# thawro/pytorch-human-pose

Measured on AMD Instinct MI355X. Metric: images/sec (fwd+decode) HigherHRNet-W32 512px, higher is better.
Workload: dtype bf16; 1 GPU; HigherHRNet-W32 inference bf16, batch 32 @ 512x512 per GPU (conv fwd on N(0,1) images + AE decode on constructed maps, 10 people/image, det_thr 0.05, tag_thr 0.5, adjust+refine); global_batch=32, parallelism=image-sharded replicas x1, no data-path collective

## Files before the change

include/hhrnet.h:

```cpp
#ifndef HHRNET_H
#define HHRNET_H
#include <stdint.h>

#ifdef __cplusplus
extern "C" {
#endif

#define HH_ABI_VERSION 3
#define HH_DTYPE_BF16 1
#define HH_DTYPE_FP8 2
#define HH_DTYPE_F16 3

typedef struct hh_net hh_net;
typedef struct hh_decoder hh_decoder;

int hh_abi_version(void);
const char *hh_last_error(void);

hh_net *hh_create(int num_kpts, int C, int dtype);
void hh_destroy(hh_net *net);

hh_net *hh_create_classifier(int C, int num_classes, int dtype);
int hh_forward_classifier(hh_net *net, const float *images, int B, int H, int W, float *logits, void *stream);

int hh_num_params(const hh_net *net);
const char *hh_param_name(const hh_net *net, int index);
int hh_param_shape(const hh_net *net, int index, int64_t shape[4]);

int hh_load_weights(hh_net *net, const char *name, const float *host, const int64_t *shape, int ndim);
int hh_finalize(hh_net *net);

int hh_calibrate(hh_net *net, const float *images, int B, int H, int W, int rounds, void *stream);

int hh_e4m3_encode(const float *x, int64_t n, unsigned char *out);
int hh_e4m3_decode(const unsigned char *x, int64_t n, float *out);

int hh_reserve(hh_net *net, int B, int H, int W);
int64_t hh_workspace_bytes(const hh_net *net);

int hh_forward(hh_net *net, const float *images, int B, int H, int W, float *init_heatmaps, float *deconv_heatmaps,
               int use_graph, void *stream);

int hh_set_multi_lane(hh_net *net, int enable);

int hh_debug_check_plan(const hh_net *net);

double hh_forward_flops(const hh_net *net, int B, int H, int W);

int hh_profile_enable(hh_net *net, int enable);
int hh_profile_count(const hh_net *net);
int hh_profile_get(hh_net *net, int index, int *cfg, double *flops, double *bytes, float *ms, float *kernel_ms, const char **layer);
int hh_profile_clock(hh_net *net, int index, double *ghz);
int hh_conv_config(int cfg, int out[7]);
int hh_conv_config_double_buffered(int cfg);

int hh_debug_conv_bench(int cfg, int B, int Hin, int Win, int cin, int cout, int with_res, int relu, int iters,
                        float *ms_per_launch, unsigned long long *stamps16, int ref_cfg, float *max_diff);

int hh_debug_bb_bench(int B, int H, int W, int iters, float *ms_per_launch, unsigned long long *stamps64);
int hh_debug_bb_compare(int B, int H, int W, int iters, float *max_diff, float *ms_classic, float *ms_pc);

int hh_debug_bb_cover(int B, int H, int W, int tall, int num_cus, int64_t counts[4]);

int hh_set_taps(hh_net *net, int enable);
int hh_num_taps(const hh_net *net);
const char *hh_tap_name(const hh_net *net, int index);
int hh_tap_shape(const hh_net *net, int index, int64_t shape[4]);
int hh_tap_read(hh_net *net, int index, float *host_nchw);

int hh_preprocess_u8(const unsigned char *image_hwc, int h, int w, const double dst_to_src[6], float *out_nchw, int H, int W,
                     const float mean[3], const float stdv[3], void *stream);

typedef struct hh_image_desc {
    long long offset;
    int h, w;
    double dst_to_src[6];
} hh_image_desc;
int hh_preprocess_u8_batch(const unsigned char *images_base, const hh_image_desc *descs_dev, int n, float *out_nchw, int H, int W,
                           const float mean[3], const float stdv[3], void *stream);

int hh_flip_images(const float *images, float *out, int B, int C, int H, int W, void *stream);
int hh_flip_merge(float *hm, int64_t hm_bstride, const float *hm_flipped, int64_t hmf_bstride, const float *tags_flipped,
                  int64_t tf_bstride, float *tags_out, int64_t to_bstride, const int32_t *perm_host, int B, int K,
                  int h, int w, void *stream);

hh_decoder *hh_decoder_create(int num_kpts, int max_people, double det_thr, double tag_thr);
void hh_decoder_destroy(hh_decoder *dec);
int hh_decoder_reserve(hh_decoder *dec, int B, int H, int W, int E);
int hh_decoder_set_exact_topk(hh_decoder *dec, int enable);

#define HH_DECODE_FALLBACK 1
#define HH_DECODE_SOLVER_GUARD 2
int hh_decode(hh_decoder *dec, const float *hm_q, int64_t hm_q_bstride, const float *hm_h, int64_t hm_h_bstride,
              const float *const *tags_q, const int64_t *tags_bstride, int E, int B, int hq, int wq, int adjust,
              int refine, float *joints, float *scores, int32_t *num_people, int32_t *flags, void *stream);

int hh_parse(hh_decoder *dec, const float *hm_full, const float *tags_full, int E, int B, int H, int W, int adjust,
             int refine, float *joints, float *scores, int32_t *num_people, int32_t *flags, void *stream);

int hh_loss_heatmaps(const float *pred, int64_t pred_bstride, const float *target, const float *mask, int B, int K, int h, int w,
                     float *loss, float *grad, int64_t grad_bstride, double *scratch, void *stream);
int hh_loss_ae_grouping(const float *tags, int64_t tags_bstride, const int32_t *joints, const int32_t *num_people, int B, int P, int K,
                        int h, int w, float *push_pull, float *grad, int64_t grad_bstride, float push_scale, float pull_scale,
                        double *scratch, void *stream);

#define HH_TRAIN_MAX_STAGES 4
typedef struct hh_train_desc {
    long long image_offset, mask_offset;
    int h, w;
    int flip, reserved;
    double image_dst_to_src[6];
    double mask_dst_to_src[HH_TRAIN_MAX_STAGES][6];
} hh_train_desc;
int hh_train_images_u8_batch(const unsigned char *batch_base, const hh_train_desc *descs_dev, int n, float *out_nchw, int H, int W,
                             const float mean[3], const float stdv[3], void *stream);
int hh_train_masks_u8_batch(const unsigned char *batch_base, const hh_train_desc *descs_dev, int n, int nstages, const int *stage_hw,
                            float *const *out, void *stream);
#define HH_MOSAIC_MAX_S 8192
typedef struct hh_mosaic_tile {
    long long image_offset, mask_offset;
    int h, w;
} hh_mosaic_tile;
typedef struct hh_mosaic_desc {
    hh_mosaic_tile tile[4];
    long long canvas_image_offset, canvas_mask_offset;
} hh_mosaic_desc;
int hh_mosaic_u8_batch(unsigned char *batch_base, const hh_mosaic_desc *descs_dev, const hh_mosaic_desc *descs_host, int n, int S,
                       void *stream);
typedef struct hh_crowd_mask_desc {
    long long mask_offset;
    int h, w;
    int seg_first, seg_count;
} hh_crowd_mask_desc;
typedef struct hh_crowd_seg_desc {
    long long toggle_offset;
    int count;
    int col_first, col_last;
    int reserved;
} hh_crowd_seg_desc;
long long hh_crowd_polygon_capacity(const double *xy, int k, int h, int w);
long long hh_crowd_polygon_toggles(const double *xy, int k, int h, int w, unsigned int *out, long long capacity);
int hh_crowd_masks_u8_batch(unsigned char *batch_base, const hh_crowd_mask_desc *descs_dev, const hh_crowd_seg_desc *segs_dev,
                            const hh_crowd_mask_desc *descs_host, const hh_crowd_seg_desc *segs_host, const unsigned char *host_base, int n,
                            int num_segs, void *stream);
int hh_crowd_mask_config(int out[4]);
// ... 403 lines not shown
```

pytorch-human-pose_amd/csrc/capi.cpp:

```cpp
#include <algorithm>
#include <cmath>
#include <cstdint>
#include <cstring>
#include <string>
#include <vector>

#include "../../include/hhrnet.h"
#include "engine.h"
#include "optim_math.h"
#include "grad_stats_math.h"
#include "ema_math.h"
#include "render_math.h"
#include "text_math.h"
#include "seg_overlay_math.h"
#include "panel_math.h"
#include "coco_eval_math.h"
#include "pose_score_math.h"
#include "cls_score_math.h"
#include "crowd_mask_math.h"
#include "track_math.h"
#include "jpeg_math.h"
#include "jpeg_dec_math.h"

const char *hh_get_error();
// ... 65 lines not shown
}
void hh_destroy(hh_net *net) { delete net; }

int hh_num_params(const hh_net *net) { return (int)net->params.size(); }
const char *hh_param_name(const hh_net *net, int i) { return (i >= 0 && i < (int)net->params.size()) ? net->params[i].name.c_str() : nullptr; }
int hh_param_shape(const hh_net *net, int i, int64_t shape[4])
{
    if (i < 0 || i >= (int)net->params.size()) return -1;
    const auto &s = net->params[i].shape;
    for (size_t d = 0; d < s.size(); ++d) shape[d] = s[d];
    return (int)s.size();
}

int hh_load_weights(hh_net *net, const char *name, const float *host, const int64_t *shape, int ndim)
{
    auto it = net->param_index.find(name);
    if (it == net->param_index.end()) { hh_set_error(std::string("hh_load_weights: unexpected key ") + name); return 1; }
    ParamSlot &p = net->params[it->second];
    if (p.counter) { p.loaded = true; return 0; }
    if (ndim != (int)p.shape.size()) { hh_set_error(std::string("hh_load_weights: rank mismatch for ") + name); return 1; }
    size_t n = 1;
    for (int d = 0; d < ndim; ++d) {
        if (shape[d] != p.shape[d]) { hh_set_error(std::string("hh_load_weights: size mismatch for ") + name); return 1; }
        n *= (size_t)shape[d];
    }
    p.data.assign(host, host + n);
    p.loaded = true;
    net->finalized = false;
    return 0;
}
int hh_e4m3_encode(const float *x, int64_t n, unsigned char *out)
{
    for (int64_t i = 0; i < n; ++i) out[i] = hh_f32_to_e4m3(x[i]);
    return 0;
}
int hh_e4m3_decode(const unsigned char *x, int64_t n, float *out)
{
    for (int64_t i = 0; i < n; ++i) out[i] = hh_e4m3_to_f32(x[i]);
    return 0;
}
int hh_finalize(hh_net *net) { return net->finalize(); }
int hh_calibrate(hh_net *net, const float *images, int B, int H, int W, int rounds, void *stream)
{
    if (!images || B <= 0 || H <= 0 || W <= 0 || H % 32 || W % 32) { hh_set_error("hh_calibrate: need images [B,3,H,W] with H, W multiples of 32"); return 1; }
    return net->calibrate(images, B, H, W, rounds > 0 ? rounds : 2, (hipStream_t)stream);
}
int hh_reserve(hh_net *net, int B, int H, int W) { return net->reserve(B, H, W); }
int64_t hh_workspace_bytes(const hh_net *net) { return net->ws_bytes; }

int hh_forward(hh_net *net, const float *images, int B, int H, int W, float *init_heatmaps, float *deconv_heatmaps,
               int use_graph, void *stream)
{
    if (net->kind != 0) { hh_set_error("hh_forward: classifier handle, use hh_forward_classifier"); return 1; }
    if (!images || !init_heatmaps || !deconv_heatmaps) { hh_set_error("hh_forward: null buffer"); return 1; }
    if (B <= 0 || H <= 0 || W <= 0 || H % 32 || W % 32) { hh_set_error("hh_forward: H and W must be positive multiples of 32"); return 1; }
    return net->forward(images, B, H, W, init_heatmaps, deconv_heatmaps, use_graph, (hipStream_t)stream);
}
double hh_forward_flops(const hh_net *net, int B, int H, int W) { return net->flops(B, H, W); }

int hh_set_multi_lane(hh_net *net, int enable)
{
    net->multi_lane = enable != 0;
    for (auto &g : net->graphs) hipGraphExecDestroy(g.exec);
    net->graphs.clear();
    return 0;
}
int hh_set_taps(hh_net *net, int enable) { net->taps_enabled = enable != 0; return 0; }
int hh_num_taps(const hh_net *net) { return (int)net->taps.size(); }
const char *hh_tap_name(const hh_net *net, int i) { return (i >= 0 && i < (int)net->taps.size()) ? net->taps[i].name.c_str() : nullptr; }
int hh_tap_shape(const hh_net *net, int i, int64_t shape[4])
{
    if (i < 0 || i >= (int)net->taps.size()) return 1;
    const TensorDesc &d = net->tensors[net->taps[i].tensor];
    shape[0] = net->lastB; shape[1] = net->taps[i].C; shape[2] = net->lastH >> d.shift; shape[3] = net->lastW >> d.shift;
    return 0;
}
int hh_tap_read(hh_net *net, int index, float *host_nchw) { return hh_tap_read_impl(net, index, host_nchw); }

int hh_debug_check_plan(const hh_net *net)
{
    std::string why;
    if (net->check_plan(&why)) { hh_set_error("schedule hazard: " + why); return 1; }
    return 0;
}

int hh_profile_enable(hh_net *net, int enable) { net->prof_enabled = enable != 0; net->prof_clk = enable == 2; net->prof_used = 0; return 0; }
int hh_profile_count(const hh_net *net) { return (int)net->prof_used; }
int hh_profile_get(hh_net *net, int i, int *cfg, double *flops, double *bytes, float *ms, float *kernel_ms, const char **layer)
{
    if (i < 0 || i >= (int)net->prof_used) { hh_set_error("hh_profile_get: index out of range"); return 1; }
    const ProfRecord &r = net->prof[i];
    HH_CHECK_HIP(hipEventSynchronize(r.e1));
    HH_CHECK_HIP(hipEventElapsedTime(ms, r.e0, r.e1));
    *cfg = r.cfg; *flops = r.flops; *bytes = r.bytes;
    *layer = net->layers[net->ops[r.op].layer].conv.c_str();
    *kernel_ms = -1.f;
    if (r.slot >= 0 && net->prof_clk && net->d_clk && net->clk_khz > 0) {
        unsigned long long t[2];
        HH_CHECK_HIP(hipMemcpy(t, net->d_clk + 4 * r.slot, 16, hipMemcpyDeviceToHost));
        if (t[1] > t[0]) *kernel_ms = (float)((double)(t[1] - t[0]) / net->clk_khz);
    }
    return 0;
}
int hh_profile_clock(hh_net *net, int i, double *ghz)
{
    if (i < 0 || i >= (int)net->prof_used) { hh_set_error("hh_profile_clock: index out of range"); return 1; }
    const ProfRecord &r = net->prof[i];
    *ghz = 0.0;
    if (r.slot >= 0 && net->prof_clk && net->d_clk && net->clk_khz > 0) {
        unsigned long long t[2];
        HH_CHECK_HIP(hipEventSynchronize(r.e1));
        HH_CHECK_HIP(hipMemcpy(t, net->d_clk + 4 * r.slot + 2, 16, hipMemcpyDeviceToHost));
        if (t[1]) *ghz = (double)t[0] / (double)t[1] * net->clk_khz * 1e-6;
    }
    return 0;
}
int hh_conv_config(int cfg, int out[7])
{
    if (cfg >= 1000 && cfg - 1000 < conv_fp8_num_configs()) {
        const Fp8ConvConfig &c = conv_fp8_config(cfg - 1000);
        out[0] = c.KS; out[1] = c.S; out[2] = c.KC; out[3] = c.NT; out[4] = 1; out[5] = c.PT; out[6] = c.TW;
        return 0;
    }
    if (cfg < 0 || cfg >= conv_num_configs()) return 1;
    const ConvConfig &c = conv_config(cfg);
    out[0] = c.KS; out[1] = c.S; out[2] = c.KC; out[3] = c.NT; out[4] = c.WC; out[5] = c.PT; out[6] = c.TW;
    return 0;
}

int hh_conv_config_double_buffered(int cfg)
{
    if (cfg >= 1000 && cfg - 1000 < conv_fp8_num_configs()) return 0;
    if (cfg < 0 || cfg >= conv_num_configs()) return -1;
    return conv_config(cfg).DB;
}

int hh_preprocess_u8(const unsigned char *image_hwc, int h, int w, const double dst_to_src[6], float *out_nchw, int H, int W,
                     const float mean[3], const float stdv[3], void *stream)
{
    if (!image_hwc || !out_nchw || h <= 0 || w <= 0 || H <= 0 || W <= 0) { hh_set_error("hh_preprocess_u8: bad argument"); return 1; }
    HH_CHECK_HIP(launch_preprocess(image_hwc, h, w, dst_to_src, out_nchw, H, W, mean, stdv, (hipStream_t)stream));
    return 0;
}

int hh_preprocess_u8_batch(const unsigned char *images_base, const hh_image_desc *descs_dev, int n, float *out_nchw, int H, int W,
                           const float mean[3], const float stdv[3], void *stream)
{
    if (!images_base || !descs_dev || !out_nchw || n <= 0 || n > 65535 || H <= 0 || W <= 0) { hh_set_error("hh_preprocess_u8_batch: bad argument"); return 1; }
    HH_CHECK_HIP(launch_preprocess_batch(images_base, descs_dev, n, out_nchw, H, W, mean, stdv,
                                         (hipStream_t)stream));
    return 0;
}

int hh_train_images_u8_batch(const unsigned char *batch_base, const hh_train_desc *descs_dev, int n, float *out_nchw, int H, int W,
                             const float mean[3], const float stdv[3], void *stream)
{
    if (!batch_base || !descs_dev || !out_nchw || !mean || !stdv) { hh_set_error("hh_train_images_u8_batch: null pointer"); return 1; }
    if (n <= 0 || n > 65535 || H <= 0 || W <= 0 || (int64_t)H * W > (1 << 30)) { hh_set_error("hh_train_images_u8_batch: need 0 < n <= 65535 and 0 < H * W <= 2^30"); return 1; }
    HH_CHECK_HIP(launch_train_images(batch_base, descs_dev, n, out_nchw, H, W, mean, stdv, (hipStream_t)stream));
    return 0;
}

int hh_train_masks_u8_batch(const unsigned char *batch_base, const hh_train_desc *descs_dev, int n, int nstages, const int *stage_hw,
                            float *const *out, void *stream)
{
    if (!batch_base || !descs_dev || !stage_hw || !out) { hh_set_error("hh_train_masks_u8_batch: null pointer"); return 1; }
// ... 2205 lines not shown
```

pytorch-human-pose_amd/csrc/kernels.h:

```cpp
#pragma once
#include <hip/hip_runtime.h>
#include <stdint.h>

#include <hip/hip_ext.h>

#include "../../include/hhrnet.h"

typedef uint16_t bf16_raw;

struct LaunchProbe { hipEvent_t start = nullptr, stop = nullptr; };
LaunchProbe &hh_launch_probe();
#define HH_LAUNCH(kernel, grid, block, lds, stream, ...)                                                            \
    do {                                                                                                            \
        LaunchProbe &lp_ = hh_launch_probe();                                                                       \
        if (lp_.start) {                                                                                            \
            hipExtLaunchKernelGGL(kernel, grid, block, lds, stream, lp_.start, lp_.stop, 0, __VA_ARGS__);           \
            lp_ = LaunchProbe{};                                                                                    \
        } else {                                                                                                    \
            hipLaunchKernelGGL(kernel, grid, block, lds, stream, __VA_ARGS__);                                      \
        }                                                                                                           \
    } while (0)

struct ConvParams {
    const bf16_raw *in;
// ... 125 lines not shown
    float *fin_out;
    int fin_K;
    unsigned long long *stamps;
    unsigned long long *clk;
};
constexpr int BBPC_TH = 14, BBPC_TW = 32;
struct BBGeom { int b, oy0, ox0; };
__host__ __device__ inline int bbpc_band(int i, int ntiles, unsigned grid)
{
    return ((ntiles & 7) == 0 && (grid & 7) == 0) ? (i & 7) * (ntiles >> 3) + (i >> 3) : i;
}
__host__ __device__ __forceinline__ BBGeom bbpc_geom(int tb, int tiles_x, int tiles_per_img, int VH)
{
    const int u = tb / tiles_per_img, tt = tb % tiles_per_img;
    const int oy = (tt / tiles_x) * BBPC_TH, bq = oy / VH;
    return BBGeom{u + bq, oy - bq * VH, (tt % tiles_x) * BBPC_TW};
}
__host__ __device__ __forceinline__ int bbpc_rowmap(int b, int y, int B, int H, int VH)
{
    const bool wrap = y >= VH;
    const int ya = wrap ? y - VH : y, bb = wrap ? b + 1 : b;
    return (((unsigned)ya < (unsigned)H) & (bb < B)) ? bb * H + ya : -1;
}
__host__ __device__ inline bool bbpc_patch_wrap(int yy, int VH) { return yy >= VH; }
__host__ __device__ inline bool bbpc_patch_row(int yy, bool wrap, bool next, int H, int VH)
{
    return ((unsigned)(wrap ? yy - VH : yy) < (unsigned)H) & (!wrap | next);
}
bool bbpc_cover(int B, int H, int W, int tall, int num_cus, long long counts[4]);

#define HH_PROF_SLOTS 1024
#define HH_CFG_BB_FUSED 100
hipError_t bb_fused_init();
hipError_t bb_fused_launch(BBParams p, int num_cus, hipStream_t s);
hipError_t bbpc_init();
bool bbpc_supported(const BBParams &p);
bool bbpc_final_supported(const BBParams &p);
hipError_t bbpc_launch(BBParams p, int num_cus, hipStream_t s, int act_dtype = 0);
#define HH_CFG_BB64_FUSED 103
hipError_t bb64_fused_init();
hipError_t bb64_fused_launch(BBParams p, int num_cus, hipStream_t s, int act_dtype = 0);

struct JuncParams {
    const bf16_raw *t2; int t2_cs;
    const bf16_raw *res; int res_cs;
    const bf16_raw *x; int x_cs;
    const bf16_raw *t2a; int t2a_cs;
    const bf16_raw *w3a; const float *b3a;
    const bf16_raw *w3, *wd, *w1;
    const float *b3, *bd, *b1;
    bf16_raw *y; int y_cs;
    bf16_raw *t1; int t1_cs;
    int npix;
    unsigned long long *clk;
};
#define HH_CFG_JUNCTION 101
hipError_t junction_init();
hipError_t junction_launch(const JuncParams &p, int num_cus, hipStream_t s, int act_dtype = 0);

struct StemParams {
    const float *images;
    const bf16_raw *w;
    const float *bias;
    bf16_raw *out; int out_cs;
    int B, H, W;
    unsigned long long *clk;
    unsigned char *out_fp8;
    float out_inv_scale;
    unsigned *absmax;
};
#define HH_CFG_STEM 102
hipError_t stem_conv_launch(const StemParams &p, hipStream_t s);
struct StemFusedParams {
    const float *images;
    const bf16_raw *w1;
    const float *b1;
    const bf16_raw *w2;
    const float *b2;
    bf16_raw *out; int out_cs;
    int B, H, W;
    unsigned long long *clk;
};
#define HH_CFG_STEM_FUSED 106
hipError_t stem_fused_init();
bool stem_fused_supported(const StemFusedParams &p);
hipError_t stem_fused_launch(const StemFusedParams &p, int num_cus, hipStream_t s, int act_dtype = 0);


struct UpAddParams {
    const bf16_raw *base; int base_cs, base_coff;
    const bf16_raw *up[3]; int up_cs[3]; int up_shift[3]; int nup;
    bf16_raw *out; int out_cs, out_coff;
    int B, H, W, C, relu;
};
hipError_t launch_upadd(const UpAddParams &p, hipStream_t s, int act_dtype = 0);
struct FusionUpParams {
    const bf16_raw *x0; int x0_cs;
    const bf16_raw *src[3];
    int src_cs[3];
    const bf16_raw *w[3];
    const float *bias[3];
    int nsrc;
    bf16_raw *out; int out_cs;
    int B, H, W;
    int tiles_x, tiles_y;
    unsigned long long *clk;
};
#define HH_CFG_FUSION_UP 107
bool fusion_up_supported(int C, int nsrc);
hipError_t fusion_up_launch(FusionUpParams p, hipStream_t s, int act_dtype = 0);
hipError_t launch_upadd_backward(const bf16_raw *dy, const bf16_raw *out, int relu, int B, int H, int W, int C, bf16_raw *g, bf16_raw *const *dup,
                                 const int *up_shift, int nup, hipStream_t s, int act_dtype = 0);
struct UpAddFp8Params {
    const unsigned char *base; int base_cs; float base_scale;
    const unsigned char *up[3]; int up_cs[3]; int up_shift[3]; float up_scale[3]; int nup;
    const bf16_raw *base16; int base16_cs;
    const bf16_raw *up16[3]; int up16_cs[3];
    unsigned char *out; int out_cs;
    float out_inv_scale;
    bf16_raw *out16; int out16_cs;
    int B, H, W, C, relu;
    unsigned *absmax;
};
hipError_t launch_upadd_fp8(const UpAddFp8Params &p, hipStream_t s);
hipError_t launch_quant_fp8(const bf16_raw *in, int in_cs, unsigned char *out, int out_cs, size_t npix, int C, float inv_scale, unsigned *absmax,
                            hipStream_t s);

hipError_t launch_lds_poison(int num_cus, hipStream_t s);
hipError_t launch_avgpool(const bf16_raw *in, int in_cs, float *out, int B, int HW, int C, hipStream_t s, int act_dtype = 0);
hipError_t launch_linear(const float *x, const float *w, const float *bias, float *y, int B, int K, int N, hipStream_t s);
hipError_t launch_avgpool_backward(const float *g, bf16_raw *dx, int B, int HW, int C, hipStream_t s, int act_dtype = 0);
hipError_t launch_linear_backward(const float *x, const float *w, const float *dy, int B, int K, int N, float *dx, float *dw, float *db,
                                  hipStream_t s);
static_assert(sizeof(hh_xent_result) == 16, "ABI 3");
hipError_t launch_softmax_xent(const float *logits, const long long *targets, int B, int N, float *dlogits, hh_xent_result *result, hipStream_t s);

static_assert(sizeof(hh_image_desc) == 64, "ABI 3");
hipError_t launch_preprocess_batch(const unsigned char *base, const hh_image_desc *descs, int n, float *out, int H, int W,
                                   const float mean[3], const float stdv[3], hipStream_t s);
hipError_t launch_warp_affine_u8(const unsigned char *img, int h, int w, const double inv[6], unsigned char *out, int H, int W, hipStream_t s);
hipError_t launch_preprocess(const unsigned char *img, int h, int w, const double inv[6], float *out, int H, int W,
                             const float mean[3], const float stdv[3], hipStream_t s);
static_assert(sizeof(hh_train_desc) == 272, "ABI 3");
struct TrainMaskStages { float *out[HH_TRAIN_MAX_STAGES]; int h[HH_TRAIN_MAX_STAGES], w[HH_TRAIN_MAX_STAGES], n; };
hipError_t launch_train_images(const unsigned char *base, const hh_train_desc *descs, int n, float *out, int H, int W, const float mean[3],
                               const float stdv[3], hipStream_t s);
hipError_t launch_train_masks(const unsigned char *base, const hh_train_desc *descs, int n, const TrainMaskStages &st, hipStream_t s);
static_assert(sizeof(hh_crop_desc) == 56, "ABI 3");
hipError_t launch_resized_crop(const unsigned char *base, const hh_crop_desc *descs, int n, float *out, int H, int W, const float mean[3],
                               const float stdv[3], hipStream_t s);
static_assert(sizeof(hh_mosaic_tile) == 24 && sizeof(hh_mosaic_desc) == 112, "ABI 3");
hipError_t launch_mosaic(unsigned char *base, const hh_mosaic_desc *descs, int n, int S, hipStream_t s);
hipError_t launch_render_poses(unsigned char *base, const hh_render_desc *descs, const hh_render_prim *prims, int n, int max_tiles, hipStream_t s);
void render_debug_host(const unsigned char *src, unsigned char *dst, const hh_render_desc &d, const hh_render_prim *prims);
hipError_t launch_resize_u8(const unsigned char *src, int h, int w, int channels, unsigned char *dst, int H, int W, hipStream_t s);
hipError_t launch_resize_u8_scaled(const unsigned char *src, int h, int w, int channels, unsigned char *dst, int H, int W, double fx, double fy, hipStream_t s);
hipError_t launch_text_labels(unsigned char *base, const hh_text_desc *descs, const hh_text_prim *prims, const uint8_t *atlas, const void *tiles,
                              long long num_tiles, hipStream_t s);
void text_debug_host(unsigned char *frame, const hh_text_desc &d, const hh_text_prim *prims, const uint8_t *atlas, const void *tiles, long long num_tiles);
hipError_t launch_seg_overlay(unsigned char *base, const hh_seg_desc *descs, const int32_t *shapes, const unsigned int *toggles, int n, int max_tiles, hipStream_t s);
hipError_t launch_jpeg_encode(unsigned char *base, const hh_jpeg_desc *descs, int n, int max_mcus, int max_rows, unsigned char *ws, int32_t *lengths,
                              hipStream_t s);
template <class Desc>
hipError_t launch_jpeg_decode(unsigned char *base, const Desc *descs, int n, int max_seg, int max_blk, int max_h, int max_w, unsigned char *ws,
                              int32_t *status, hipStream_t s);
hipError_t launch_jpeg_index(unsigned char *base, const hh_jpeg_dec_desc *descs, int n, int mps, int subseq_bytes, int32_t *status, hipStream_t s);
// ... 96 lines not shown
```

pytorch-human-pose_amd/csrc/stem_fused.hip:

```cpp
#include "mfma_dev.h"

namespace {
constexpr int T2H = 2, T2W = 32;
constexpr int MR = 2 * T2H + 1, MC = 2 * T2W + 1;
constexpr int MPIX = MR * MC, NQ = (MPIX + 31) / 32;
constexpr int PRW = 4 * T2H + 3, PCW = 4 * T2W + 3;
constexpr int PLANE = PRW * PCW, NVAL = 3 * PLANE;
constexpr int NLD = (NVAL + 255) / 256;
constexpr int PS2 = 144, HALF = (MC + 1) / 2;
constexpr int MID_BYTES = MR * 2 * HALF * PS2;
constexpr int PATCH_BYTES = ((NVAL + 1) * 2 + 15) / 16 * 16;
constexpr int OFF_PATCH = MID_BYTES, OFF_BIAS = OFF_PATCH + PATCH_BYTES, LDS_BYTES = OFF_BIAS + 2 * 64 * 4;
constexpr int RD = 3, NFB = RD + 1;
}

template <typename E>
__global__ __launch_bounds__(256, 1) void stem_fused_kernel(const StemFusedParams p)
{
    extern __shared__ __attribute__((aligned(16))) char smem[];
    unsigned short *patch = reinterpret_cast<unsigned short *>(smem + OFF_PATCH);
    const int tid = threadIdx.x;
    if (p.clk && tid == 0) atomicMin(p.clk, wall_clock64());
    const int lds0 = (int)(size_t)(__attribute__((address_space(3))) char *)smem;
    const int wave = __builtin_amdgcn_readfirstlane(tid >> 6), lane = tid & 63, r = lane & 31, h = lane >> 5;
    const int H1 = p.H >> 1, W1 = p.W >> 1, H2 = p.H >> 2, W2 = p.W >> 2;
    const size_t img_elems = (size_t)3 * p.H * p.W, out_elems = (size_t)H2 * W2 * p.out_cs;
    constexpr unsigned OOB = 0x80000000u;

    const int row2 = wave >> 1, ct2 = wave & 1;
    u32x4 a1[2][2];
#pragma unroll
    for (int ct = 0; ct < 2; ++ct)
#pragma unroll
        for (int kk = 0; kk < 2; ++kk) a1[ct][kk] = reinterpret_cast<const u32x4 *>(p.w1)[((ct * 2 + kk) * 2 + h) * 32 + r];
    u32x4 w2r[36];
    {
        const auto rs_w = __builtin_amdgcn_make_buffer_rsrc(const_cast<bf16_raw *>(p.w2), 0, 9 * 8 * 64 * 16, 0x00020000);
        static_for<36>([&](auto fc) {
            constexpr int f = decltype(fc)::value, tap = f >> 2, kk = f & 3;
            w2r[f] = __builtin_bit_cast(u32x4, __builtin_amdgcn_raw_buffer_load_b128(rs_w, (((tap * 8 + kk * 2 + h) * 64) + ct2 * 32 + r) * 16, 0, 0));
        });
    }
    if (tid < 64) {
        reinterpret_cast<float *>(smem + OFF_BIAS)[tid] = p.b1[tid];
        reinterpret_cast<float *>(smem + OFF_BIAS)[64 + tid] = p.b2[tid];
    }
    if (tid == 0) patch[NVAL] = 0;
    auto bias_acc = [&](int off) {
        f32x16 b0;
#pragma unroll
        for (int q = 0; q < 4; ++q) {
            const float4 bv = *reinterpret_cast<const float4 *>(smem + OFF_BIAS + (off + 8 * q + 4 * h) * 4);
            b0[4 * q + 0] = bv.x; b0[4 * q + 1] = bv.y; b0[4 * q + 2] = bv.z; b0[4 * q + 3] = bv.w;
        }
        return b0;
    };

    const int tiles_x = (W2 + T2W - 1) / T2W, tiles_y = (H2 + T2H - 1) / T2H, ntiles = p.B * tiles_x * tiles_y;
    struct Geom { int b, oy0, ox0; };
    auto geom = [&](int t) {
        const int tx = t % tiles_x, ty = (t / tiles_x) % tiles_y;
        return Geom{t / (tiles_x * tiles_y), ty * T2H, tx * T2W};
    };
    float pv[NLD];
    auto patch_load = [&](int t) {
        const bool on = t < ntiles;
        const Geom g = geom(on ? t : 0);
        const auto rs_img = __builtin_amdgcn_make_buffer_rsrc(const_cast<float *>(p.images + (size_t)g.b * img_elems), 0, (int)(img_elems * 4), 0x00020000);
        const int iy0 = 4 * g.oy0 - 3, ix0 = 4 * g.ox0 - 3;
#pragma unroll
        for (int it = 0; it < NLD; ++it) {
            const int i = tid + 256 * it;
            const int c = i / PLANE, rem = i - c * PLANE, py = rem / PCW, px = rem - py * PCW;
            const int iy = iy0 + py, ix = ix0 + px;
            const bool ok = on & (i < NVAL) & ((unsigned)iy < (unsigned)p.H) & ((unsigned)ix < (unsigned)p.W);
            const unsigned voff = ok ? (unsigned)(((c * p.H + iy) * p.W + ix) * 4) : OOB;
            pv[it] = __builtin_bit_cast(float, __builtin_amdgcn_raw_buffer_load_b32(rs_img, (int)voff, 0, 0));
        }
    };
    auto patch_write = [&]() {
#pragma unroll
        for (int it = 0; it < NLD; ++it) {
            const int i = tid + 256 * it;
            if (it + 1 < NLD || i < NVAL) patch[i] = E::cvt(pv[it]);
        }
    };
    int off[2][8];
#pragma unroll
    for (int kk = 0; kk < 2; ++kk)
#pragma unroll
        for (int j = 0; j < 8; ++j) {
            const int t = kk * 16 + 8 * h + j;
            off[kk][j] = t < 27 ? (t / 9) * PLANE + ((t % 9) / 3) * PCW + (t % 3) : -1;
        }

    int t = blockIdx.x;
    patch_load(t);
    patch_write();
    __syncthreads();

    for (; t < ntiles; t += gridDim.x) {
        const Geom g = geom(t);
        patch_load(t + (int)gridDim.x);

        constexpr int NQW = (NQ + 3) / 4;
        u32x4 bf[NQW][2];
#pragma unroll
        for (int qi = 0; qi < NQW; ++qi) {
            const int q = wave + 4 * qi;
            const int m = q * 32 + r, mc = m < MPIX ? m : MPIX - 1;
            const int my = mc / MC, mx = mc - my * MC;
            const int base = (2 * my) * PCW + 2 * mx;
#pragma unroll
            for (int kk = 0; kk < 2; ++kk) {
                unsigned short v[8];
#pragma unroll
                for (int j = 0; j < 8; ++j) v[j] = patch[off[kk][j] >= 0 ? base + off[kk][j] : NVAL];
                bf[qi][kk] = u32x4{(unsigned)v[0] | ((unsigned)v[1] << 16), (unsigned)v[2] | ((unsigned)v[3] << 16),
                                   (unsigned)v[4] | ((unsigned)v[5] << 16), (unsigned)v[6] | ((unsigned)v[7] << 16)};
            }
        }
        const f32x16 bias1[2] = {bias_acc(0), bias_acc(32)};
#pragma unroll
        for (int qi = 0; qi < NQW; ++qi) {
            const int q = wave + 4 * qi;
            if (q >= NQ) break;
            const int m = q * 32 + r, mc = m < MPIX ? m : MPIX - 1;
            const int my = mc / MC, mx = mc - my * MC;
            const int gy = 2 * g.oy0 - 1 + my, gx = 2 * g.ox0 - 1 + mx;
            const bool inside = ((unsigned)gy < (unsigned)H1) & ((unsigned)gx < (unsigned)W1);
            char *dst = smem + ((my * 2 + (mx & 1)) * HALF + (mx >> 1)) * PS2 + h * 16;
#pragma unroll
            for (int ct = 0; ct < 2; ++ct) {
                f32x16 acc = bias1[ct];
#pragma unroll
                for (int kk = 0; kk < 2; ++kk)
                    acc = E::mfma(a1[ct][kk], bf[qi][kk], acc);
                u32x4 o[2];
                pack_rows16<E>(acc, o);
                if (m < MPIX) {
                    *reinterpret_cast<u32x4 *>(dst + ct * 64) = inside ? o[0] : u32x4{0u, 0u, 0u, 0u};
                    *reinterpret_cast<u32x4 *>(dst + ct * 64 + 32) = inside ? o[1] : u32x4{0u, 0u, 0u, 0u};
                }
            }
        }
        __syncthreads();

        patch_write();

        {
            f32x16 acc = bias_acc(64 + ct2 * 32);
            const int ma = lds0 + (row2 * 4 * HALF + r) * PS2 + h * 16;
            u32x4 fb[NFB];
            auto ldb = [&](auto sc, int buf) {
                constexpr int s = decltype(sc)::value, tap = s >> 2, kk = s & 3, ky = tap / 3, kx = tap % 3;
                fb[buf] = lds_read_async<((ky * 2 + (kx & 1)) * HALF + (kx >> 1)) * PS2 + kk * 32>(ma);
            };
            static_for<RD>([&](auto sc) { ldb(sc, decltype(sc)::value); });
            static_for<36>([&](auto sc) {
                constexpr int s = decltype(sc)::value;
                if constexpr (s + RD < 36) ldb(std::integral_constant<int, s + RD>{}, (s + RD) % NFB);
                lds_wait<(35 - s < RD ? 35 - s : RD)>(fb[s % NFB]);
                acc = E::mfma(w2r[s], fb[s % NFB], acc);
            });
            u32x4 o[2];
            pack_rows16<E>(acc, o);
            const int oy = g.oy0 + row2, ox = g.ox0 + r;
            const bool ok = (oy < H2) & (ox < W2);
            const auto rs_out = __builtin_amdgcn_make_buffer_rsrc(p.out + (size_t)g.b * out_elems, 0, (int)(out_elems * 2), 0x00020000);
            const unsigned voff = ok ? (unsigned)(((oy * W2 + ox) * p.out_cs + ct2 * 32 + 8 * h) * 2) : OOB;
            __builtin_amdgcn_raw_buffer_store_b128(o[0], rs_out, (int)voff, 0, 0);
            __builtin_amdgcn_raw_buffer_store_b128(o[1], rs_out, (int)voff, 32, 0);
        }
        __syncthreads();
    }
    if (p.clk && tid == 0) atomicMax(p.clk + 1, wall_clock64());
}

hipError_t stem_fused_init()
{
    const hipError_t e = hipFuncSetAttribute(reinterpret_cast<const void *>(stem_fused_kernel<ElemBF16>), hipFuncAttributeMaxDynamicSharedMemorySize, LDS_BYTES);
    if (e != hipSuccess) return e;
    return hipFuncSetAttribute(reinterpret_cast<const void *>(stem_fused_kernel<ElemF16>), hipFuncAttributeMaxDynamicSharedMemorySize, LDS_BYTES);
}

bool stem_fused_supported(const StemFusedParams &p)
{
    return p.H % 4 == 0 && p.W % 4 == 0 && (size_t)3 * p.H * p.W * 4 < 0x7fffffffull && (size_t)(p.H / 4) * (p.W / 4) * p.out_cs * 2 < 0x7fffffffull;
}

hipError_t stem_fused_launch(const StemFusedParams &p, int num_cus, hipStream_t s, int act_dtype)
{
    if (act_dtype != 0 && act_dtype != 1) return hipErrorInvalidValue;
    const int H2 = p.H >> 2, W2 = p.W >> 2;
    const int ntiles = p.B * ((H2 + T2H - 1) / T2H) * ((W2 + T2W - 1) / T2W);
    const int grid = ntiles < num_cus ? ntiles : num_cus;
    if (act_dtype) HH_LAUNCH(stem_fused_kernel<ElemF16>, dim3(grid), dim3(256), LDS_BYTES, s, p);
    else HH_LAUNCH(stem_fused_kernel<ElemBF16>, dim3(grid), dim3(256), LDS_BYTES, s, p);
    return hipGetLastError();
}
```

Before: 7079 images/sec.

## Warp-specialize fused stem into producer and consumer waves with double-buffered LDS

Rewrites the fused stem conv kernel to use 512 threads. Four producer waves stage the image patch with 128-bit loads and compute the first stride-2 conv into a double-buffered mid tile, while four consumer waves run the second conv on the previous tile. This overlaps global loads, the first conv and the second conv across tiles instead of serialising them with block-wide barriers. It also adds a debug entry point and optional timestamp probes. The cost is double the LDS footprint and a one-tile pipeline skew, and the stem is only a small part of the whole network.

```diff
diff --git a/include/hhrnet.h b/include/hhrnet.h
--- a/include/hhrnet.h
+++ b/include/hhrnet.h
@@ -61,6 +61,8 @@
 int hh_debug_bb_compare(int B, int H, int W, int iters, float *max_diff, float *ms_classic, float *ms_pc);
 
 int hh_debug_bb_cover(int B, int H, int W, int tall, int num_cus, int64_t counts[4]);
+
+int hh_debug_stem_fused(hh_net *net, const float *images, int B, int H, int W, void *out16, void *stream);
 
 int hh_set_taps(hh_net *net, int enable);
 int hh_num_taps(const hh_net *net);
diff --git a/pytorch-human-pose_amd/csrc/capi.cpp b/pytorch-human-pose_amd/csrc/capi.cpp
--- a/pytorch-human-pose_amd/csrc/capi.cpp
+++ b/pytorch-human-pose_amd/csrc/capi.cpp
@@ -171,6 +171,26 @@
     std::string why;
     if (net->check_plan(&why)) { hh_set_error("schedule hazard: " + why); return 1; }
     return 0;
+}
+
+int hh_debug_stem_fused(hh_net *net, const float *images, int B, int H, int W, void *out16, void *stream)
+{
+    if (!net->finalized) { hh_set_error("hh_debug_stem_fused: call hh_finalize first"); return 1; }
+    if (!images || !out16 || B <= 0 || H <= 0 || W <= 0) { hh_set_error("hh_debug_stem_fused: null buffer or empty shape"); return 1; }
+    for (const Op &op : net->ops) {
+        if (op.kind != OP_STEM || op.layer2 < 0) continue;
+        const ConvLayer &l = net->layers[op.layer], &l2 = net->layers[op.layer2];
+        StemFusedParams q{};
+        q.images = images; q.w1 = l.d_w; q.b1 = l.d_bias; q.w2 = l2.d_w; q.b2 = l2.d_bias;
+        q.out = (bf16_raw *)out16; q.out_cs = 64;
+        q.B = B; q.H = H; q.W = W;
+        if (!stem_fused_supported(q)) { hh_set_error("hh_debug_stem_fused: H, W must be multiples of 4 and an image below 2 GB"); return 1; }
+        if (net->sw.poison_lds) HH_CHECK_HIP(launch_lds_poison(net->num_cus, (hipStream_t)stream));
+        HH_CHECK_HIP(stem_fused_launch(q, net->num_cus, (hipStream_t)stream, net->act()));
+        return 0;
+    }
+    hh_set_error("hh_debug_stem_fused: the handle's plan has no fused stem (HH_NO_STEM_FUSED, or an fp8 handle)");
+    return 1;
 }
 
 int hh_profile_enable(hh_net *net, int enable) { net->prof_enabled = enable != 0; net->prof_clk = enable == 2; net->prof_used = 0; return 0; }
diff --git a/pytorch-human-pose_amd/csrc/kernels.h b/pytorch-human-pose_amd/csrc/kernels.h
--- a/pytorch-human-pose_amd/csrc/kernels.h
+++ b/pytorch-human-pose_amd/csrc/kernels.h
@@ -231,6 +231,23 @@
     unsigned long long *clk;
 };
 #define HH_CFG_STEM_FUSED 106
+constexpr int STEM_T2H = 2, STEM_T2W = 32;
+constexpr int STEM_PROWS = 4 * STEM_T2H + 3;
+constexpr int STEM_PVEC = (4 * STEM_T2W + 4 + 4) / 4;
+constexpr int STEM_PRS = 4 * STEM_PVEC;
+constexpr int STEM_STAGE_THREADS = 256, STEM_ROUND_ROWS = STEM_STAGE_THREADS / STEM_PVEC;
+constexpr int STEM_ROUNDS = (3 * STEM_PROWS + STEM_ROUND_ROWS - 1) / STEM_ROUND_ROWS;
+struct StemUnit { int c, py, v; bool act; };
+__host__ __device__ inline StemUnit stem_unit(int tid, int round)
+{
+    const int rr = tid / STEM_PVEC, row = STEM_ROUND_ROWS * round + rr, c = row / STEM_PROWS;
+    return StemUnit{c, row - c * STEM_PROWS, tid - rr * STEM_PVEC, rr < STEM_ROUND_ROWS && row < 3 * STEM_PROWS};
+}
+__host__ __device__ inline int stem_unit_goff(const StemUnit &u, int H, int W) { return (u.c * H + u.py) * W + 4 * u.v; }
+__host__ __device__ inline int stem_tile_origin(int oy0, int ox0, int W) { return (4 * oy0 - 3) * W + 4 * ox0 - 4; }
+__host__ __device__ inline int stem_unit_slot(const StemUnit &u) { return (u.c * STEM_PROWS + u.py) * STEM_PRS + 4 * u.v; }
+__host__ __device__ inline bool stem_unit_row_ok(int py, int oy0, int H) { return (unsigned)(4 * oy0 - 3 + py) < (unsigned)H; }
+__host__ __device__ inline bool stem_unit_col_ok(int v, int ox0, int W) { return (unsigned)(4 * ox0 - 4 + 4 * v) < (unsigned)W; }
 hipError_t stem_fused_init();
 bool stem_fused_supported(const StemFusedParams &p);
 hipError_t stem_fused_launch(const StemFusedParams &p, int num_cus, hipStream_t s, int act_dtype = 0);
diff --git a/pytorch-human-pose_amd/csrc/stem_fused.hip b/pytorch-human-pose_amd/csrc/stem_fused.hip
--- a/pytorch-human-pose_amd/csrc/stem_fused.hip
+++ b/pytorch-human-pose_amd/csrc/stem_fused.hip
@@ -1,51 +1,58 @@
 #include "mfma_dev.h"
 
 namespace {
-constexpr int T2H = 2, T2W = 32;
+constexpr int T2H = STEM_T2H, T2W = STEM_T2W;
 constexpr int MR = 2 * T2H + 1, MC = 2 * T2W + 1;
 constexpr int MPIX = MR * MC, NQ = (MPIX + 31) / 32;
-constexpr int PRW = 4 * T2H + 3, PCW = 4 * T2W + 3;
-constexpr int PLANE = PRW * PCW, NVAL = 3 * PLANE;
-constexpr int NLD = (NVAL + 255) / 256;
+constexpr int NQW = (NQ + 3) / 4;
+constexpr int PRS = STEM_PRS, PLANE = STEM_PROWS * PRS, NVAL = 3 * PLANE;
+constexpr int GBASE_MAX = 2 * (MR - 1) * PRS + 2 * (MC - 1) + 1, NZPAD = (GBASE_MAX + 1 + 7) / 8 * 8;
+constexpr int NROUND = STEM_ROUNDS, ROUND_BYTES = STEM_ROUND_ROWS * PRS * 2;
 constexpr int PS2 = 144, HALF = (MC + 1) / 2;
 constexpr int MID_BYTES = MR * 2 * HALF * PS2;
-constexpr int PATCH_BYTES = ((NVAL + 1) * 2 + 15) / 16 * 16;
-constexpr int OFF_PATCH = MID_BYTES, OFF_BIAS = OFF_PATCH + PATCH_BYTES, LDS_BYTES = OFF_BIAS + 2 * 64 * 4;
+constexpr int PATCH_BYTES = (NVAL + NZPAD) * 2;
+constexpr int OFF_PATCH = 2 * MID_BYTES, OFF_BIAS = OFF_PATCH + 2 * PATCH_BYTES, OFF_TRASH = OFF_BIAS + 2 * 64 * 4;
+constexpr int LDS_BYTES = OFF_TRASH + 32 * PS2;
+constexpr int NTHR = 512;
 constexpr int RD = 3, NFB = RD + 1;
-}
+static_assert(MID_BYTES % 16 == 0 && PATCH_BYTES % 16 == 0 && (NVAL * 2) % 16 == 0 && NZPAD % 8 == 0, "16-byte LDS units");
+static_assert(STEM_STAGE_THREADS == NTHR / 2 && NROUND * STEM_ROUND_ROWS >= 3 * STEM_PROWS, "the producers stage the whole patch");
+static_assert(LDS_BYTES <= 160 * 1024, "LDS");
+}
+
+#ifdef HH_STAMP
+__device__ unsigned long long g_stem_stamps[72];
+#define PSTAMP(i) do { if (blockIdx.x == 0 && it == 2 && lane == 0) g_stem_stamps[wave * 8 + (i)] = __builtin_amdgcn_s_memtime(); } while (0)
+extern "C" int hh_debug_stem_stamps(unsigned long long *out) { return (int)hipMemcpyFromSymbol(out, HIP_SYMBOL(g_stem_stamps), sizeof(g_stem_stamps)); }
+#else
+#define PSTAMP(i)
+#endif
 
 template <typename E>
-__global__ __launch_bounds__(256, 1) void stem_fused_kernel(const StemFusedParams p)
+__global__ __launch_bounds__(NTHR, 1) void stem_fused_kernel(const StemFusedParams p)
 {
     extern __shared__ __attribute__((aligned(16))) char smem[];
-    unsigned short *patch = reinterpret_cast<unsigned short *>(smem + OFF_PATCH);
     const int tid = threadIdx.x;
     if (p.clk && tid == 0) atomicMin(p.clk, wall_clock64());
+#ifdef HH_STAMP
+    if (blockIdx.x == 0 && tid == 0) { g_stem_stamps[64] = __builtin_amdgcn_s_memtime(); g_stem_stamps[65] = __builtin_amdgcn_s_memrealtime(); }
+#endif
     const int lds0 = (int)(size_t)(__attribute__((address_space(3))) char *)smem;
     const int wave = __builtin_amdgcn_readfirstlane(tid >> 6), lane = tid & 63, r = lane & 31, h = lane >> 5;
+    const bool producer = wave < 4;
+    const int wj = wave & 3;
     const int H1 = p.H >> 1, W1 = p.W >> 1, H2 = p.H >> 2, W2 = p.W >> 2;
     const size_t img_elems = (size_t)3 * p.H * p.W, out_elems = (size_t)H2 * W2 * p.out_cs;
     constexpr unsigned OOB = 0x80000000u;
 
-    const int row2 = wave >> 1, ct2 = wave & 1;
-    u32x4 a1[2][2];
-#pragma unroll
-    for (int ct = 0; ct < 2; ++ct)
-#pragma unroll
-        for (int kk = 0; kk < 2; ++kk) a1[ct][kk] = reinterpret_cast<const u32x4 *>(p.w1)[((ct * 2 + kk) * 2 + h) * 32 + r];
-    u32x4 w2r[36];
-    {
-        const auto rs_w = __builtin_amdgcn_make_buffer_rsrc(const_cast<bf16_raw *>(p.w2), 0, 9 * 8 * 64 * 16, 0x00020000);
-        static_for<36>([&](auto fc) {
-            constexpr int f = decltype(fc)::value, tap = f >> 2, kk = f & 3;
-            w2r[f] = __builtin_bit_cast(u32x4, __builtin_amdgcn_raw_buffer_load_b128(rs_w, (((tap * 8 + kk * 2 + h) * 64) + ct2 * 32 + r) * 16, 0, 0));
-        });
-    }
     if (tid < 64) {
         reinterpret_cast<float *>(smem + OFF_BIAS)[tid] = p.b1[tid];
         reinterpret_cast<float *>(smem + OFF_BIAS)[64 + tid] = p.b2[tid];
     }
-    if (tid == 0) patch[NVAL] = 0;
+    if (tid >= 64 && tid < 64 + 2 * (NZPAD / 8)) {
+        const int z = tid - 64, buf = z / (NZPAD / 8), k = z - buf * (NZPAD / 8);
+        *reinterpret_cast<u32x4 *>(smem + OFF_PATCH + buf * PATCH_BYTES + NVAL * 2 + k * 16) = u32x4{0u, 0u, 0u, 0u};
+    }
     auto bias_acc = [&](int off) {
         f32x16 b0;
 #pragma unroll
@@ -57,124 +64,186 @@
     };
 
     const int tiles_x = (W2 + T2W - 1) / T2W, tiles_y = (H2 + T2H - 1) / T2H, ntiles = p.B * tiles_x * tiles_y;
-    struct Geom { int b, oy0, ox0; };
-    auto geom = [&](int t) {
-        const int tx = t % tiles_x, ty = (t / tiles_x) % tiles_y;
-        return Geom{t / (tiles_x * tiles_y), ty * T2H, tx * T2W};
+    const int nloc = (ntiles - (int)blockIdx.x + (int)gridDim.x - 1) / (int)gridDim.x;
+    struct Geom { int b, ty, tx; };
+    auto split = [&](int t) { return Geom{t / (tiles_x * tiles_y), (t / tiles_x) % tiles_y, t % tiles_x}; };
+    const Geom g_first = split((int)blockIdx.x), g_step = split((int)gridDim.x);
+    auto advance = [&](Geom g) {
+        g.tx += g_step.tx;
+        if (g.tx >= tiles_x) { g.tx -= tiles_x; ++g.ty; }
+        g.ty += g_step.ty;
+        if (g.ty >= tiles_y) { g.ty -= tiles_y; ++g.b; }
+        g.b += g_step.b;
+        return g;
     };
-    float pv[NLD];
-    auto patch_load = [&](int t) {
-        const bool on = t < ntiles;
-        const Geom g = geom(on ? t : 0);
-        const auto rs_img = __builtin_amdgcn_make_buffer_rsrc(const_cast<float *>(p.images + (size_t)g.b * img_elems), 0, (int)(img_elems * 4), 0x00020000);
-        const int iy0 = 4 * g.oy0 - 3, ix0 = 4 * g.ox0 - 3;
-#pragma unroll
-        for (int it = 0; it < NLD; ++it) {
-            const int i = tid + 256 * it;
-            const int c = i / PLANE, rem = i - c * PLANE, py = rem / PCW, px = rem - py * PCW;
-            const int iy = iy0 + py, ix = ix0 + px;
-            const bool ok = on & (i < NVAL) & ((unsigned)iy < (unsigned)p.H) & ((unsigned)ix < (unsigned)p.W);
-            const unsigned voff = ok ? (unsigned)(((c * p.H + iy) * p.W + ix) * 4) : OOB;
-            pv[it] = __builtin_bit_cast(float, __builtin_amdgcn_raw_buffer_load_b32(rs_img, (int)voff, 0, 0));
-        }
-    };
-    auto patch_write = [&]() {
-#pragma unroll
-        for (int it = 0; it < NLD; ++it) {
-            const int i = tid + 256 * it;
-            if (it + 1 < NLD || i < NVAL) patch[i] = E::cvt(pv[it]);
-        }
-    };
-    int off[2][8];
-#pragma unroll
-    for (int kk = 0; kk < 2; ++kk)
-#pragma unroll
-        for (int j = 0; j < 8; ++j) {
-            const int t = kk * 16 + 8 * h + j;
-            off[kk][j] = t < 27 ? (t / 9) * PLANE + ((t % 9) / 3) * PCW + (t % 3) : -1;
-        }
-
-    int t = blockIdx.x;
-    patch_load(t);
-    patch_write();
-    __syncthreads();
-
-    for (; t < ntiles; t += gridDim.x) {
-        const Geom g = geom(t);
-        patch_load(t + (int)gridDim.x);
-
-        constexpr int NQW = (NQ + 3) / 4;
-        u32x4 bf[NQW][2];
+
+    if (producer) {
+        u32x4 a1[2][2];
+#pragma unroll
+        for (int ct = 0; ct < 2; ++ct)
+#pragma unroll
+            for (int kk = 0; kk < 2; ++kk) a1[ct][kk] = reinterpret_cast<const u32x4 *>(p.w1)[((ct * 2 + kk) * 2 + h) * 32 + r];
+
+        int gp[NROUND];
+        const StemUnit u0 = stem_unit(tid, 0);
+        const int st_v = u0.v, st_slot = stem_unit_slot(u0) * 2;
+#pragma unroll
+        for (int i = 0; i < NROUND; ++i) {
+            const StemUnit u = stem_unit(tid, i);
+            gp[i] = u.act ? (stem_unit_goff(u, p.H, p.W) * 4) | u.py : -1;
+        }
+        u32x4 pv[NROUND];
+        auto patch_load = [&](const Geom &g) {
+            const int oy0 = g.ty * T2H, ox0 = g.tx * T2W;
+            const auto rs_img = __builtin_amdgcn_make_buffer_rsrc(const_cast<float *>(p.images + (size_t)g.b * img_elems), 0, (int)(img_elems * 4), 0x00020000);
+            const int origin = stem_tile_origin(oy0, ox0, p.W) * 4;
+            const bool xok = stem_unit_col_ok(st_v, ox0, p.W);
+            static_for<NROUND>([&](auto ic) {
+                constexpr int i = decltype(ic)::value;
+                const bool ok = (gp[i] >= 0) & xok & stem_unit_row_ok(gp[i] & 15, oy0, p.H);
+                const unsigned voff = ok ? (unsigned)(origin + (gp[i] & ~15)) : OOB;
+                pv[i] = __builtin_bit_cast(u32x4, __builtin_amdgcn_raw_buffer_load_b128(rs_img, (int)voff, 0, 0));
+            });
+        };
+        auto patch_write = [&](int buf) {
+            char *dst = smem + OFF_PATCH + buf * PATCH_BYTES + st_slot;
+            static_for<NROUND>([&](auto ic) {
+                constexpr int i = decltype(ic)::value;
+                if (gp[i] >= 0) {
+                    const unsigned w0 = pv[i][0], w1 = pv[i][1], w2 = pv[i][2], w3 = pv[i][3];
+                    const unsigned lo = E::round2(__uint_as_float(w0), __uint_as_float(w1)), hi = E::round2(__uint_as_float(w2), __uint_as_float(w3));
+                    *reinterpret_cast<u32x2 *>(dst + i * ROUND_BYTES) = u32x2{lo, hi};
+                }
+            });
+        };
+        int off[2][8];
+#pragma unroll
+        for (int kk = 0; kk < 2; ++kk)
+#pragma unroll
+            for (int j = 0; j < 8; ++j) {
+                const int t = kk * 16 + 8 * h + j;
+                off[kk][j] = (t < 27 ? (t / 9) * PLANE + ((t % 9) / 3) * PRS + (t % 3) : NVAL) * 2;
+            }
+        int gbase[NQW], mdst[NQW], myx[NQW];
 #pragma unroll
         for (int qi = 0; qi < NQW; ++qi) {
-            const int q = wave + 4 * qi;
-            const int m = q * 32 + r, mc = m < MPIX ? m : MPIX - 1;
+            const int m = (wj + 4 * qi) * 32 + r, mc = m < MPIX ? m : MPIX - 1;
             const int my = mc / MC, mx = mc - my * MC;
-            const int base = (2 * my) * PCW + 2 * mx;
-#pragma unroll
-            for (int kk = 0; kk < 2; ++kk) {
-                unsigned short v[8];
-#pragma unroll
-                for (int j = 0; j < 8; ++j) v[j] = patch[off[kk][j] >= 0 ? base + off[kk][j] : NVAL];
-                bf[qi][kk] = u32x4{(unsigned)v[0] | ((unsigned)v[1] << 16), (unsigned)v[2] | ((unsigned)v[3] << 16),
-                                   (unsigned)v[4] | ((unsigned)v[5] << 16), (unsigned)v[6] | ((unsigned)v[7] << 16)};
+            gbase[qi] = ((2 * my) * PRS + 2 * mx + 1) * 2;
+            mdst[qi] = m < MPIX ? ((my * 2 + (mx & 1)) * HALF + (mx >> 1)) * PS2 + h * 16 : -1;
+            myx[qi] = my | (mx << 8);
+        }
+        char *const trash = smem + OFF_TRASH + r * PS2 + h * 16;
+
+        Geom g = g_first, gn = advance(g_first);
+        patch_load(g);
+        patch_write(0);
+        lds_barrier();
+
+        for (int it = 0; it <= nloc; ++it) {
+            PSTAMP(0);
+            if (it < nloc) {
+                const bool more = it + 1 < nloc;
+                if (more) patch_load(gn);
+                PSTAMP(1);
+                const int oy0 = g.ty * T2H, ox0 = g.tx * T2W;
+                const unsigned short *patch = reinterpret_cast<const unsigned short *>(smem + OFF_PATCH + (it & 1) * PATCH_BYTES);
+                char *mid = smem + (it & 1) * MID_BYTES;
+
+                u32x4 bf[NQW][2];
+#pragma unroll
+                for (int qi = 0; qi < NQW; ++qi)
+#pragma unroll
+                    for (int kk = 0; kk < 2; ++kk) {
+                        unsigned short v[8];
+#pragma unroll
+                        for (int j = 0; j < 8; ++j) v[j] = *reinterpret_cast<const unsigned short *>(reinterpret_cast<const char *>(patch) + gbase[qi] + off[kk][j]);
+                        bf[qi][kk] = u32x4{(unsigned)v[0] | ((unsigned)v[1] << 16), (unsigned)v[2] | ((unsigned)v[3] << 16),
+                                           (unsigned)v[4] | ((unsigned)v[5] << 16), (unsigned)v[6] | ((unsigned)v[7] << 16)};
+                    }
+                const f32x16 bias1[2] = {bias_acc(0), bias_acc(32)};
+                f32x16 acc[NQW][2];
+#pragma unroll
+                for (int kk = 0; kk < 2; ++kk)
+#pragma unroll
+                    for (int qi = 0; qi < NQW; ++qi)
+#pragma unroll
+                        for (int ct = 0; ct < 2; ++ct) acc[qi][ct] = E::mfma(a1[ct][kk], bf[qi][kk], kk == 0 ? bias1[ct] : acc[qi][ct]);
+#pragma unroll
+                for (int qi = 0; qi < NQW; ++qi) {
+                    const int my = myx[qi] & 255, mx = myx[qi] >> 8;
+                    const int gy = 2 * oy0 - 1 + my, gx = 2 * ox0 - 1 + mx;
+                    const bool inside = ((unsigned)gy < (unsigned)H1) & ((unsigned)gx < (unsigned)W1);
+                    char *dst = mdst[qi] >= 0 ? mid + mdst[qi] : trash;
+#pragma unroll
+                    for (int ct = 0; ct < 2; ++ct) {
+                        u32x4 o[2];
+                        pack_rows16<E>(acc[qi][ct], o);
+                        *reinterpret_cast<u32x4 *>(dst + ct * 64) = inside ? o[0] : u32x4{0u, 0u, 0u, 0u};
+                        *reinterpret_cast<u32x4 *>(dst + ct * 64 + 32) = inside ? o[1] : u32x4{0u, 0u, 0u, 0u};
+                    }
+                }
+                PSTAMP(2);
+                if (more) patch_write((it + 1) & 1);
+                g = gn;
+                gn = advance(gn);
             }
-        }
-        const f32x16 bias1[2] = {bias_acc(0), bias_acc(32)};
-#pragma unroll
-        for (int qi = 0; qi < NQW; ++qi) {
-            const int q = wave + 4 * qi;
-            if (q >= NQ) break;
-            const int m = q * 32 + r, mc = m < MPIX ? m : MPIX - 1;
-            const int my = mc / MC, mx = mc - my * MC;
-            const int gy = 2 * g.oy0 - 1 + my, gx = 2 * g.ox0 - 1 + mx;
-            const bool inside = ((unsigned)gy < (unsigned)H1) & ((unsigned)gx < (unsigned)W1);
-            char *dst = smem + ((my * 2 + (mx & 1)) * HALF + (mx >> 1)) * PS2 + h * 16;
-#pragma unroll
-            for (int ct = 0; ct < 2; ++ct) {
-                f32x16 acc = bias1[ct];
-#pragma unroll
-                for (int kk = 0; kk < 2; ++kk)
-                    acc = E::mfma(a1[ct][kk], bf[qi][kk], acc);
+            PSTAMP(3);
+            lds_barrier();
+            PSTAMP(4);
+        }
+    } else {
+        const int row2 = wj >> 1, ct2 = wj & 1;
+        u32x4 w2r[36];
+        {
+            const auto rs_w = __builtin_amdgcn_make_buffer_rsrc(const_cast<bf16_raw *>(p.w2), 0, 9 * 8 * 64 * 16, 0x00020000);
+            static_for<36>([&](auto fc) {
+                constexpr int f = decltype(fc)::value, tap = f >> 2, kk = f & 3;
+                w2r[f] = __builtin_bit_cast(u32x4, __builtin_amdgcn_raw_buffer_load_b128(rs_w, (((tap * 8 + kk * 2 + h) * 64) + ct2 * 32 + r) * 16, 0, 0));
+            });
+        }
+        const int ma0 = lds0 + (row2 * 4 * HALF + r) * PS2 + h * 16;
+        Geom g = g_first;
+        lds_barrier();
+
+        for (int it = 0; it <= nloc; ++it) {
+            PSTAMP(0);
+            if (it >= 1) {
+                f32x16 acc = bias_acc(64 + ct2 * 32);
+                PSTAMP(1);
+                const int ma = ma0 + ((it - 1) & 1) * MID_BYTES;
+                u32x4 fb[NFB];
+                auto ldb = [&](auto sc, int buf) {
+                    constexpr int s = decltype(sc)::value, tap = s >> 2, kk = s & 3, ky = tap / 3, kx = tap % 3;
+                    fb[buf] = lds_read_async<((ky * 2 + (kx & 1)) * HALF + (kx >> 1)) * PS2 + kk * 32>(ma);
+                };
+                static_for<RD>([&](auto sc) { ldb(sc, decltype(sc)::value); });
+                static_for<36>([&](auto sc) {
+                    constexpr int s = decltype(sc)::value;
+                    if constexpr (s + RD < 36) ldb(std::integral_constant<int, s + RD>{}, (s + RD) % NFB);
+                    lds_wait<(35 - s < RD ? 35 - s : RD)>(fb[s % NFB]);
+                    acc = E::mfma(w2r[s], fb[s % NFB], acc);
+                });
+                PSTAMP(2);
                 u32x4 o[2];
                 pack_rows16<E>(acc, o);
-                if (m < MPIX) {
-                    *reinterpret_cast<u32x4 *>(dst + ct * 64) = inside ? o[0] : u32x4{0u, 0u, 0u, 0u};
-                    *reinterpret_cast<u32x4 *>(dst + ct * 64 + 32) = inside ? o[1] : u32x4{0u, 0u, 0u, 0u};
-                }
+                const int oy = g.ty * T2H + row2, ox = g.tx * T2W + r;
+                const bool ok = (oy < H2) & (ox < W2);
+                const auto rs_out = __builtin_amdgcn_make_buffer_rsrc(p.out + (size_t)g.b * out_elems, 0, (int)(out_elems * 2), 0x00020000);
+                const unsigned voff = ok ? (unsigned)(((oy * W2 + ox) * p.out_cs + ct2 * 32 + 8 * h) * 2) : OOB;
+                __builtin_amdgcn_raw_buffer_store_b128(o[0], rs_out, (int)voff, 0, 0);
+                __builtin_amdgcn_raw_buffer_store_b128(o[1], rs_out, (int)voff, 32, 0);
+                g = advance(g);
             }
-        }
-        __syncthreads();
-
-        patch_write();
-
-        {
-            f32x16 acc = bias_acc(64 + ct2 * 32);
-            const int ma = lds0 + (row2 * 4 * HALF + r) * PS2 + h * 16;
-            u32x4 fb[NFB];
-            auto ldb = [&](auto sc, int buf) {
-                constexpr int s = decltype(sc)::value, tap = s >> 2, kk = s & 3, ky = tap / 3, kx = tap % 3;
-                fb[buf] = lds_read_async<((ky * 2 + (kx & 1)) * HALF + (kx >> 1)) * PS2 + kk * 32>(ma);
-            };
-            static_for<RD>([&](auto sc) { ldb(sc, decltype(sc)::value); });
-            static_for<36>([&](auto sc) {
-                constexpr int s = decltype(sc)::value;
-                if constexpr (s + RD < 36) ldb(std::integral_constant<int, s + RD>{}, (s + RD) % NFB);
-                lds_wait<(35 - s < RD ? 35 - s : RD)>(fb[s % NFB]);
-                acc = E::mfma(w2r[s], fb[s % NFB], acc);
-            });
-            u32x4 o[2];
-            pack_rows16<E>(acc, o);
-            const int oy = g.oy0 + row2, ox = g.ox0 + r;
-            const bool ok = (oy < H2) & (ox < W2);
-            const auto rs_out = __builtin_amdgcn_make_buffer_rsrc(p.out + (size_t)g.b * out_elems, 0, (int)(out_elems * 2), 0x00020000);
-            const unsigned voff = ok ? (unsigned)(((oy * W2 + ox) * p.out_cs + ct2 * 32 + 8 * h) * 2) : OOB;
-            __builtin_amdgcn_raw_buffer_store_b128(o[0], rs_out, (int)voff, 0, 0);
-            __builtin_amdgcn_raw_buffer_store_b128(o[1], rs_out, (int)voff, 32, 0);
-        }
-        __syncthreads();
+            PSTAMP(3);
+            lds_barrier();
+            PSTAMP(4);
+        }
     }
     if (p.clk && tid == 0) atomicMax(p.clk + 1, wall_clock64());
+#ifdef HH_STAMP
+    if (blockIdx.x == 0 && tid == 0) { g_stem_stamps[66] = __builtin_amdgcn_s_memtime(); g_stem_stamps[67] = __builtin_amdgcn_s_memrealtime(); }
+#endif
 }
 
 hipError_t stem_fused_init()
@@ -195,7 +264,7 @@
     const int H2 = p.H >> 2, W2 = p.W >> 2;
     const int ntiles = p.B * ((H2 + T2H - 1) / T2H) * ((W2 + T2W - 1) / T2W);
     const int grid = ntiles < num_cus ? ntiles : num_cus;
-    if (act_dtype) HH_LAUNCH(stem_fused_kernel<ElemF16>, dim3(grid), dim3(256), LDS_BYTES, s, p);
-    else HH_LAUNCH(stem_fused_kernel<ElemBF16>, dim3(grid), dim3(256), LDS_BYTES, s, p);
+    if (act_dtype) HH_LAUNCH(stem_fused_kernel<ElemF16>, dim3(grid), dim3(NTHR), LDS_BYTES, s, p);
+    else HH_LAUNCH(stem_fused_kernel<ElemBF16>, dim3(grid), dim3(NTHR), LDS_BYTES, s, p);
     return hipGetLastError();
 }
```

Result: faster. 7161 images/sec (median of 6 runs) (+1.2%).
